# QingzhiWang/LIS-SLAM

Measured on AMD Instinct MI355X. Metric: scan-to-submap registrations/sec (64x1800 pts, 200k submap), higher is better.
Workload: dtype f32; 1 GPU; configs[1]: batch=64 synthetic 64x1800 scans vs one shared 200k-pt submap per GPU, semantic mask off, 10 fixed GN iterations, target index build inside the step; batch_per_gpu=64, submap_points=200000, gn_iters=10, parallelism=independent batches x1 + RCCL all-gather of results

## Files before the change

### include/lisreg.h

```cpp
#ifndef LISREG_H_
#define LISREG_H_

#include <stdint.h>

#ifdef __cplusplus
extern "C" {
#endif

#define LISREG_VERSION 1

#define LISREG_OK                        0
#define LISREG_NOT_ENOUGH_FEATURES       1
#define LISREG_TOO_FEW_CORRESPONDENCES   2
#define LISREG_LEAF_TOO_SMALL            3
#define LISREG_ERR_ARG                  -1
#define LISREG_ERR_HIP                  -2
#define LISREG_ERR_NO_TARGET            -3
#define LISREG_ERR_NOMEM                -4
#define LISREG_ERR_COMM                 -5

#define LISREG_FMT_XYZI    0
#define LISREG_FMT_XYZIL   1
#define LISREG_FMT_DEVICE  2
#define LISREG_FMT_DEVICE_XYZI 4
// ... 88 lines not shown
int  lisreg_batch_prepare(lisreg_ctx* ctx, int n_items, const lisreg_item* items,
                          const lisreg_params* params, const float* T_init);
int  lisreg_batch_run(lisreg_ctx* ctx);
int  lisreg_batch_fetch(lisreg_ctx* ctx, float* T, lisreg_stats* stats);
int  lisreg_stage_host_items(lisreg_ctx* ctx, int n_items, const lisreg_item* items, lisreg_item* items_out);

void* lisreg_batch_result_device(const lisreg_ctx* ctx);

int  lisreg_set_option(lisreg_ctx* ctx, const char* name, int value);
int  lisreg_get_option(const lisreg_ctx* ctx, const char* name, int* value);

int  lisreg_get_counters(lisreg_ctx* ctx, unsigned long long* out, int n);

int  lisreg_get_neighbors(lisreg_ctx* ctx, int* out, int n_elems);

int  lisreg_test_fit_models(lisreg_ctx* ctx, int kind, int n, const float* neighbours, const float* queries,
                            const lisreg_params* params, int exact, float* out);

#define LISREG_SOLVE_STATE_STRIDE 56
int  lisreg_test_solve_steps(lisreg_ctx* ctx, int n_items, int n_steps, const int* n_rows, const double* rows,
                             const float* T_init, const int* degenerate_in, const int* n_sc, const int* n_ss,
                             const lisreg_imu* imu, const lisreg_params* params,
                             float* trace_out, float* state_out, float* results_out);

int  lisreg_get_target_index(lisreg_ctx* ctx, int slot, int kind, int* dims, float* geom,
                             float* sorted_out, int sorted_capacity, int* cell_start_out, int cell_capacity);

int  lisreg_get_target_graph(lisreg_ctx* ctx, int slot, int kind, int* k, float* rows_out, float* meta_out, int capacity_points);

int  lisreg_get_target_cell_rows(lisreg_ctx* ctx, int slot, int kind, int* n_rows, int* k, int* table_out, int capacity_cells,
                                 float* rows_out, float* meta_out, int capacity_rows);

int  lisreg_get_trace(lisreg_ctx* ctx, float* buf, int max_iters);

int  lisreg_set_profiling(lisreg_ctx* ctx, int enable);
int  lisreg_get_timing(lisreg_ctx* ctx, double out[5]);

int  lisreg_voxel_downsample(lisreg_ctx* ctx, const void* in, int n, int stride_bytes, int fmt, float leaf,
                             void* out, int out_capacity, int* n_out);
int  lisreg_voxel_downsample_multi(lisreg_ctx* ctx, int k, const void* const* in, const int* n, const float* leaf, int fmt,
                                   void* const* out, const int* out_capacity, int* n_out);
int  lisreg_transform_cloud(lisreg_ctx* ctx, const void* in, int n, int stride_bytes, int fmt, const float T[6], void* out);

#define LISREG_FMT_XYZIRT  3
typedef struct lisreg_feature_params {
    int   n_scan;
// ... 325 lines not shown
```

### lis-slam_amd/csrc/lisreg_api.hip

```cpp
#include "lisreg_ctx.hpp"

#include <dlfcn.h>

#include <algorithm>
#include <chrono>
#include <cmath>
#include <cstdio>
#include <cstdlib>
#include <cstring>
#include <string>
#include <vector>

using namespace lisreg;

namespace lisreg {
thread_local std::string g_static_err;
int ctx_fail(lisreg_ctx* c, int code, const std::string& msg)
{
    if (c) c->err = msg; else g_static_err = msg;
    return code;
}

bool ensure_side_stream(lisreg_ctx* c)
{
// ... 1349 lines not shown
    return LISREG_OK;
}

int lisreg_test_fit_models(lisreg_ctx* c, int kind, int n, const float* neighbours, const float* queries, const lisreg_params* params,
                           int exact, float* out)
{
    if (!c) return LISREG_ERR_ARG;
    if ((kind != 0 && kind != 1) || n < 0 || !params || (n > 0 && (!neighbours || !queries || !out)))
        return fail(c, LISREG_ERR_ARG, "test_fit_models: bad arguments");
    if (n == 0) return LISREG_OK;
    HIPCHK(c, hipSetDevice(c->device));
    DevBuf nb, q, o;
    HIPCHK(c, nb.ensure(sizeof(float) * 15 * (size_t)n));
    HIPCHK(c, q.ensure(sizeof(float) * 3 * (size_t)n));
    HIPCHK(c, o.ensure(sizeof(float) * 10 * (size_t)n));
    HIPCHK(c, hipMemcpyAsync(nb.p, neighbours, sizeof(float) * 15 * (size_t)n, hipMemcpyHostToDevice, c->stream));
    HIPCHK(c, hipMemcpyAsync(q.p, queries, sizeof(float) * 3 * (size_t)n, hipMemcpyHostToDevice, c->stream));
    DevParams prm = make_dev_params(*params);
    prm.exact = exact ? 1 : 0;
    if (exact) launch_test_fit_exact(kind, n, nb.as<float>(), q.as<float>(), prm, o.as<float>(), c->stream);
    else launch_test_fit(kind, n, nb.as<float>(), q.as<float>(), prm, o.as<float>(), c->stream);
    HIPCHK(c, hipGetLastError());
    HIPCHK(c, hipMemcpyAsync(out, o.p, sizeof(float) * 10 * (size_t)n, hipMemcpyDeviceToHost, c->stream));
    HIPCHK(c, hipStreamSynchronize(c->stream));
    return LISREG_OK;
}

int lisreg_test_solve_steps(lisreg_ctx* c, int n_items, int n_steps, const int* n_rows, const double* rows, const float* T_init,
                            const int* degenerate_in, const int* n_sc, const int* n_ss, const lisreg_imu* imu,
                            const lisreg_params* params, float* trace_out, float* state_out, float* results_out)
{
    if (!c) return LISREG_ERR_ARG;
    if (n_items < 0 || n_steps < 1 || n_steps > 64 || !params || (n_items > 0 && (!n_rows || !T_init)))
        return fail(c, LISREG_ERR_ARG, "test_solve_steps: bad arguments");
    if (n_items == 0) return LISREG_OK;
    size_t total_rows = 0;
    for (int i = 0; i < n_items; ++i) {
        if (n_rows[i] < 0) return fail(c, LISREG_ERR_ARG, "test_solve_steps: negative row count");
        total_rows += (size_t)n_rows[i];
    }
    if (total_rows > 0x7fffffffu || (total_rows > 0 && !rows)) return fail(c, LISREG_ERR_ARG, "test_solve_steps: bad rows");
    HIPCHK(c, hipSetDevice(c->device));
    const size_t n = (size_t)n_items;
    DevParams prm = make_dev_params(*params);
    std::vector<ItemState> h_items(n);
    memset(h_items.data(), 0, sizeof(ItemState) * n);
// ... 694 lines not shown
```

### lis-slam_amd/csrc/lisreg_index.hip

```cpp
#include "lisreg_internal.hpp"

namespace lisreg {

namespace {

constexpr int kScanBlock = 256;
constexpr int kScanItems = 8;
constexpr int kScanTile  = kScanBlock * kScanItems;

__device__ __forceinline__ int wave_incl_scan(int v, int lane)
{
#pragma unroll
    for (int d = 1; d < 64; d <<= 1) {
        int t = __shfl_up(v, d);
        if (lane >= d) v += t;
    }
    return v;
}

__device__ __forceinline__ int block_excl_scan(int v, int* total, int* s_wave )
{
    const int lane = threadIdx.x & 63, wave = threadIdx.x >> 6;
    int inc = wave_incl_scan(v, lane);
    if (lane == 63) s_wave[wave] = inc;
// ... 561 lines not shown
    if (!kLarge || n_s <= cap) {
        SlotsLds sl;
        sl.idx = (uint32_t*)(s_dyn + ucap + 1);
        sl.pos = (uint16_t*)(sl.idx + cap);
        strip_build_body<NT>(t, y0, cell0, ucells, s0, n_s, s_dyn, sl, tmp_pts, s_wave);
    } else {
        SlotsGlobal sl;
        sl.idx = g_slot_idx + s0; sl.pos = g_slot_pos + s0;
        strip_build_body<NT>(t, y0, cell0, ucells, s0, n_s, s_dyn, sl, tmp_pts, s_wave);
    }
}

constexpr int kGraphWPB = 1;
constexpr int kGraphPPW = 8;

template <int M> __device__ __forceinline__ int lane_xor(int v)
{
    if constexpr (M == 1)       return __builtin_amdgcn_mov_dpp(v, 0xB1, 0xF, 0xF, true);
    else if constexpr (M == 2)  return __builtin_amdgcn_mov_dpp(v, 0x4E, 0xF, 0xF, true);
    else if constexpr (M == 3)  return __builtin_amdgcn_mov_dpp(v, 0x1B, 0xF, 0xF, true);
    else if constexpr (M == 7)  return __builtin_amdgcn_mov_dpp(v, 0x141, 0xF, 0xF, true);
    else if constexpr (M == 15) return __builtin_amdgcn_mov_dpp(v, 0x140, 0xF, 0xF, true);
    else if constexpr (M == 8)  return __builtin_amdgcn_mov_dpp(v, 0x128, 0xF, 0xF, true);
    else return __shfl_xor(v, M);
}

__device__ __forceinline__ void graph_row_q32(const GridIndex& g, const float4 q, int hx, int hy, int hz, int s,
                                              float4* __restrict__ row_out, float2* __restrict__ meta_out, int (*s_off)[64], int (*s_js)[64]);

__device__ __forceinline__ void graph_build_wave(const GridIndex& g, int s, int (*s_off)[64], int (*s_js)[64])
{
    const float4 q = g.pts[s];
    const int hx = cell_coord(q.x, g.ox, g.inv_cell, g.nx), hy = cell_coord(q.y, g.oy, g.inv_cell, g.ny), hz = cell_coord(q.z, g.oz, g.inv_cell, g.nz);
    graph_row_q32(g, q, hx, hy, hz, s, const_cast<float4*>(g.nbr) + (size_t)s * kGraphK, const_cast<float2*>(g.nbr_meta) + s, s_off, s_js);
}

__global__ __launch_bounds__(64 * kGraphWPB) void k_graph_build_one(GridIndex g)
{
    __shared__ int s_off[kGraphWPB][64], s_js[kGraphWPB][64];
    const int first = (blockIdx.x * kGraphWPB + (threadIdx.x >> 6)) * kGraphPPW;
#pragma unroll 1
    for (int i = 0; i < kGraphPPW; ++i) {
        const int s = first + i;
        if (s >= g.n) break;
        graph_build_wave(g, s, s_off, s_js);
    }
}
// ... 139 lines not shown
    for (int dx = -2; dx <= 2; ++dx) {
        const int x = ix + dx;
        if (x < 0 || x >= g.nx) continue;
#pragma unroll
        for (int dy = -2; dy <= 2; ++dy) {
            const int y = iy + dy;
            if (y < 0 || y >= g.ny) continue;
            const int base = (x * g.ny + y) * g.nz;
            cnt5 += g.cell_start[base + z1 + 1] - g.cell_start[base + z0];
        }
    }
    const int m = omask[cid] & 255;
    const bool r = cnt5 != 0 && crow_reached(g, reach, ix, iy, iz);
    need[cid] = r ? 1 + __popc(m) : 0;
    omask[cid] = cnt5 ? (r ? (m | (min(cnt5, 0xffff) << 8)) : kCrowUnreached) : 0;
}

__global__ __launch_bounds__(256) void k_crow_classify_plain(GridIndex g, int n_cells, int* __restrict__ need, int* __restrict__ omask,
                                                             const unsigned* __restrict__ reach)
{
    crow_classify_plain_body(g, n_cells, need, omask, reach, blockIdx.x);
}

template <int M, int LowBit> __device__ __forceinline__ unsigned cmpx32(unsigned k, int lane)
{
    const unsigned pk = (unsigned)lane_xor<M>((int)k);
    const unsigned lo = min(k, pk), hi = max(k, pk);
    return (lane & LowBit) == 0 ? lo : hi;
}
template <int H> __device__ __forceinline__ unsigned half_cleaners32(unsigned k, int lane)
{
    if constexpr (H > 0) { k = cmpx32<H, H>(k, lane); return half_cleaners32<(H >> 1)>(k, lane); }
    else return k;
}
template <int H> __device__ __forceinline__ unsigned merge_blocks32(unsigned k, int lane)
{
    k = cmpx32<2 * H - 1, H>(k, lane);
    return half_cleaners32<(H >> 1)>(k, lane);
}
__device__ __forceinline__ unsigned sort64x32(unsigned k, int lane)
{
    k = merge_blocks32<1>(k, lane); k = merge_blocks32<2>(k, lane); k = merge_blocks32<4>(k, lane);
    k = merge_blocks32<8>(k, lane); k = merge_blocks32<16>(k, lane); k = merge_blocks32<32>(k, lane);
    return k;
}

template <int R>
struct CrowBlock { int x0, x1, y0, y1, z0, z1, total; };

template <int R>
__device__ __forceinline__ CrowBlock<R> crow_runs(const GridIndex& g, int hx, int hy, int hz, int (*s_off)[64], int (*s_js)[64])
{
    constexpr int W = 2 * R + 1, NR = W * W;
    static_assert(NR <= 64, "one lane per z-run");
    const int lane = threadIdx.x & 63, wave = threadIdx.x >> 6;
    CrowBlock<R> b;
    b.x0 = max(hx - R, 0); b.x1 = min(hx + R, g.nx - 1); b.y0 = max(hy - R, 0); b.y1 = min(hy + R, g.ny - 1);
    b.z0 = max(hz - R, 0); b.z1 = min(hz + R, g.nz - 1);
    int js = 0, len = 0;
    if (lane < NR) {
        const int ix = hx + lane / W - R, iy = hy + lane % W - R;
        if (ix >= b.x0 && ix <= b.x1 && iy >= b.y0 && iy <= b.y1) {
            const int base = (ix * g.ny + iy) * g.nz;
            js = g.cell_start[base + b.z0];
            len = g.cell_start[base + b.z1 + 1] - js;
        }
    }
    int inc = len;
#pragma unroll
    for (int d = 1; d < 64; d <<= 1) { const int t = __shfl_up(inc, d); if (lane >= d) inc += t; }
    b.total = __shfl(inc, 63);
    __builtin_amdgcn_wave_barrier();
    s_off[wave][lane] = inc - len; s_js[wave][lane] = js;
    __builtin_amdgcn_wave_barrier();
    return b;
}

template <int R>
__device__ __forceinline__ float crow_inscribed(const GridIndex& g, const CrowBlock<R>& b, float qx, float qy, float qz)
{
    float rc = 3.0e18f;
    if (b.x0 > 0)        rc = fminf(rc, qx - (g.ox + (float)b.x0 * g.cell));
    if (b.x1 < g.nx - 1) rc = fminf(rc, (g.ox + (float)(b.x1 + 1) * g.cell) - qx);
    if (b.y0 > 0)        rc = fminf(rc, qy - (g.oy + (float)b.y0 * g.cell));
    if (b.y1 < g.ny - 1) rc = fminf(rc, (g.oy + (float)(b.y1 + 1) * g.cell) - qy);
    if (b.z0 > 0)        rc = fminf(rc, qz - (g.oz + (float)b.z0 * g.cell));
    if (b.z1 < g.nz - 1) rc = fminf(rc, (g.oz + (float)(b.z1 + 1) * g.cell) - qz);
    return fmaxf(rc - 1e-3f, 0.f);
}

constexpr unsigned kInfQ = 0x7f800000u;

constexpr int kListQueueWaves = 4;
template <int R, bool kFilter = false>
__device__ __forceinline__ void crow_list(const GridIndex& g, const CrowBlock<R>& b, float qx, float qy, float qz,
                                          int (*s_off)[64], int (*s_js)[64], unsigned& topk, int& topi, float4& topc, bool& have_c,
                                          int exclude = -1 ,
                                          float rc2 = 3.0e38f )
{
    constexpr int W = 2 * R + 1, NR = W * W;
    const int lane = threadIdx.x & 63, wave = threadIdx.x >> 6;
    __shared__ unsigned s_qk[kListQueueWaves][128];
    __shared__ int s_qj[kListQueueWaves][128];
    topk = kInfQ; topi = -1;
    topc = make_float4(0.f, 0.f, 0.f, 0.f);
    have_c = b.total <= 64;
    auto candidate = [&](int t, int& cj, float4& cc) -> unsigned {
        unsigned ck = kInfQ;
        cj = -1; cc = make_float4(0.f, 0.f, 0.f, 0.f);
        if (t < b.total) {
            int lo = 0, hi = NR - 1;
#pragma unroll
            for (int it = 0; it < (NR > 32 ? 6 : 5); ++it) { const int mid = (lo + hi + 1) >> 1; if (s_off[wave][mid] <= t) lo = mid; else hi = mid - 1; }
            const int j = s_js[wave][lo] + (t - s_off[wave][lo]);
            const float4 c = g.pts[j];
            cc = c;
            const float ex = qx - c.x, ey = qy - c.y, ez = qz - c.z;
            const float d2 = ex * ex + ey * ey + ez * ez;
            if (j != exclude && d2 < 3.0e38f) { ck = __float_as_uint(d2) & ~0x7Fu; cj = j; }
        }
        return ck;
    };
    bool first = true;
    auto take = [&](unsigned ck_in, int cj, const float4 cc) {
        unsigned k = ck_in | (unsigned)lane;
        k = sort64x32(k, lane);
        const int cs = __shfl(cj, (int)(k & 63u));
        const unsigned ck = k & ~0x7Fu;
        if (have_c) { const int sl = (int)(k & 63u); topc = make_float4(__shfl(cc.x, sl), __shfl(cc.y, sl), __shfl(cc.z, sl), 0.f); }
        if (first) { topk = ck; topi = cs; first = false; }
        else {
            const unsigned kt = topk | 64u | (unsigned)lane;
            const unsigned kcr = (unsigned)__shfl((int)(ck | (unsigned)lane), 63 - lane);
            const unsigned m = half_cleaners32<32>(min(kt, kcr), lane);
            const int pos = (int)(m & 63u);
            const int from_top = __shfl(topi, pos), from_chunk = __shfl(cs, pos);
            topi = (m & 64u) ? from_top : from_chunk;
            topk = m & ~0x7Fu;
        }
    };
    if (!kFilter || b.total <= 64) {
#pragma unroll 1
        for (int c0 = 0; c0 < b.total; c0 += 64) {
            int cj; float4 cc;
            const unsigned ck = candidate(c0 + lane, cj, cc);
            take(ck, cj, cc);
        }
        return;
    }
    int pend = 0;
#pragma unroll 1
    for (int c0 = 0; c0 < b.total; c0 += 64) {
        int cj; float4 cc;
        const unsigned ck = candidate(c0 + lane, cj, cc);
        const bool in = cj >= 0 && __uint_as_float(ck) <= rc2;
        const unsigned long long m = __ballot(in);
        if (in) {
            const int slot = pend + (int)__builtin_amdgcn_mbcnt_hi((unsigned)(m >> 32), __builtin_amdgcn_mbcnt_lo((unsigned)m, 0u));
            s_qk[wave][slot] = ck; s_qj[wave][slot] = cj;
        }
        pend += __popcll(m);
        __builtin_amdgcn_wave_barrier();
        if (pend >= 64) {
            const unsigned qk = s_qk[wave][lane]; const int qj = s_qj[wave][lane];
            const int rest = pend - 64;
            unsigned rk = 0u; int rj = 0;
            if (lane < rest) { rk = s_qk[wave][64 + lane]; rj = s_qj[wave][64 + lane]; }
            __builtin_amdgcn_wave_barrier();
            if (lane < rest) { s_qk[wave][lane] = rk; s_qj[wave][lane] = rj; }
            pend = rest;
            __builtin_amdgcn_wave_barrier();
            take(qk, qj, make_float4(0.f, 0.f, 0.f, 0.f));
        }
    }
    if (pend > 0 || first) {
        unsigned qk = kInfQ; int qj = -1;
        if (lane < pend) { qk = s_qk[wave][lane]; qj = s_qj[wave][lane]; }
// ... 67 lines not shown
                const int oi = __shfl(keep ? topi : -1, sl);
                const float ox = __shfl(e.x, sl), oy = __shfl(e.y, sl), oz = __shfl(e.z, sl);
                const bool okeep = oi >= 0 && __uint_as_float(k & ~0x7Fu) <= rho_o2;
                const int ocnt = __popcll(__ballot(okeep));
                float4 oe = make_float4(mx, my, mz, __int_as_float(-1));
                if (okeep) oe = make_float4(ox, oy, oz, __int_as_float(oi));
                orow[lane] = oe;
                if (lane == 0) meta_out[slot] = make_float2(rho_o2, __int_as_float(ocnt));
            } else {
                unsigned ok; int oi; bool okeep; float4 oe, oc; bool ohave;
                const float orc = crow_inscribed<R>(g, b, mx, my, mz);
                crow_list<R>(g, b, mx, my, mz, s_off, s_js, ok, oi, oc, ohave, -1, orc * orc);
                (void)crow_emit(g, mx, my, mz, orc, ok, oi, orow, meta_out + slot, okeep, oe, oc, ohave);
            }
            ++slot;
        }
    }
}

constexpr int kCrowWPB = 1;
constexpr int kCrowCPW = 8;
constexpr int kCrowWaves = 6;
static_assert(kGraphWPB <= kListQueueWaves && kCrowWPB <= kListQueueWaves, "crow_list's LDS queue has one region per wavefront of a workgroup");
__device__ __forceinline__ void crow_build_body(const GridIndex& g, int n_cells, const int* __restrict__ need, int* __restrict__ omask,
                                                const int* __restrict__ scan, int cap,
                                                int blk_, int (*s_off)[64], int (*s_js)[64])
{
    const int lane = threadIdx.x & 63;
    const int first = __builtin_amdgcn_readfirstlane((blk_ * kCrowWPB + (int)(threadIdx.x >> 6)) * kCrowCPW);
    int* tab = const_cast<int*>(g.crow_tab);
    int n_l = 0, b_l = 0, om_l = 0;
    if (lane < kCrowCPW && first + lane < n_cells) {
        n_l = need[first + lane];
        om_l = omask[first + lane];
        omask[first + lane] = 0;
        if (n_l) b_l = scan[first + lane];
        const bool fits = n_l != 0 && !(b_l + n_l > cap || b_l >= (1 << 23));
        tab[first + lane] = n_l == 0 ? ((om_l & kCrowUnreached) ? -1 : -2) : (fits ? (b_l << 8) | (om_l & 255) : -1);
        if (!fits) n_l = 0;
    }
    unsigned long long live = __ballot(n_l != 0);
#pragma unroll 1
    while (live) {
        const int i = __ffsll((long long)live) - 1;
        live &= live - 1;
        const int cid = first + i;
// ... 20 lines not shown
__global__ __launch_bounds__(256) void k_crow_mark_pair(CrowJobs J, float margin_cells)
{
    const int k = (int)blockIdx.x < J.j[0].nb ? 0 : 1;
    const CrowJob& j = J.j[k];
    crow_mark_body(j.g, margin_cells * j.g.cell, j.omask, (int)blockIdx.x - (k ? J.j[0].nb : 0));
}
__global__ __launch_bounds__(256) void k_crow_classify_pair(CrowJobs J, float margin_cells)
{
    extern __shared__ int s_cs[];
    const int k = (int)blockIdx.x < J.j[0].nb ? 0 : 1;
    const CrowJob& j = J.j[k];
    const int blk = (int)blockIdx.x - (k ? J.j[0].nb : 0);
    if (j.plain) crow_classify_plain_body(j.g, j.n_cells, j.need, j.omask, j.reach, blk);
    else crow_classify_body(j.g, j.tiles_y, j.need, j.omask, j.reach, blk, s_cs, margin_cells * j.g.cell);
}
__global__ __launch_bounds__(64 * kCrowWPB) __attribute__((amdgpu_waves_per_eu(kCrowWaves, kCrowWaves))) void k_crow_build_pair(CrowJobs J)
{
    __shared__ int s_off[kCrowWPB][64], s_js[kCrowWPB][64];
    const int k = (int)blockIdx.x < J.j[0].nb ? 0 : 1;
    const CrowJob& j = J.j[k];
    crow_build_body(j.g, j.n_cells, j.need, j.omask, j.scan, j.cap, (int)blockIdx.x - (k ? J.j[0].nb : 0), s_off, s_js);
}

__global__ __launch_bounds__(kBlockQ) void k_count_jumps(const BlockDesc* __restrict__ blocks, const Segment* __restrict__ segs,
                                                         float thr2, int* __restrict__ jumps)
{
    const BlockDesc bd = blocks[blockIdx.x];
    const Segment sg = segs[bd.seg];
    const int e = bd.start + threadIdx.x;
    bool jump = false;
    if ((int)threadIdx.x < bd.count && e + 1 < sg.n) {
        const float4 a = sg.src[e], b = sg.src[e + 1];
        const float dx = a.x - b.x, dy = a.y - b.y, dz = a.z - b.z;
        jump = dx * dx + dy * dy + dz * dz > thr2;
    }
    const unsigned long long m = __ballot(jump);
    if ((threadIdx.x & 63) == 0 && m) atomicAdd(jumps, __popcll(m));
}

__global__ __launch_bounds__(256) void k_voxel_keys(const float4* __restrict__ pts, int n, VoxelDesc d,
                                                    uint32_t* __restrict__ elem_bucket, uint32_t* __restrict__ elem_sub,
                                                    int* __restrict__ hist)
{
    const int i = blockIdx.x * 256 + threadIdx.x;
    if (i >= n) return;
    const float4 p = pts[i];
// ... 569 lines not shown
    if (m.off[m.k] > 0) k_concat_jobs<<<(m.off[m.k] + 255) / 256, 256, 0, st>>>(j, m, cat);
}

__global__ void k_multi_bounds(const int* __restrict__ slot, VoxelMulti m, int* __restrict__ out)
{
    if ((int)threadIdx.x <= m.k) out[threadIdx.x] = slot[m.off[threadIdx.x]];
}
void launch_multi_bounds(const int* slot, const VoxelMulti& m, int* out, hipStream_t st) { k_multi_bounds<<<1, 64, 0, st>>>(slot, m, out); }

__global__ __launch_bounds__(256) void k_hand_out(const float4* __restrict__ src, VoxelHandOut h)
{
    const int v = blockIdx.x * 256 + threadIdx.x;
    if (v >= h.vo[h.k]) return;
    int s = 0;
#pragma unroll
    for (int j = 1; j < kVoxelMultiMax; ++j) if (j < h.k && v >= h.vo[j]) s = j;
    h.out[s][v - h.vo[s]] = src[v];
}
void launch_hand_out(const float4* src, const VoxelHandOut& h, hipStream_t st)
{
    if (h.vo[h.k] > 0) k_hand_out<<<(h.vo[h.k] + 255) / 256, 256, 0, st>>>(src, h);
}

void launch_count_jumps(const BlockDesc* blocks, int n_blocks, const Segment* segs, float thr, int* jumps, hipStream_t st)
{
    (void)hipMemsetAsync(jumps, 0, sizeof(int), st);
    if (n_blocks > 0) k_count_jumps<<<n_blocks, kBlockQ, 0, st>>>(blocks, segs, thr * thr, jumps);
}

void launch_exclusive_scan(const int* in, int* out, int* tmp, int n, hipStream_t st) { exclusive_scan(in, out, tmp, n, st); }

void launch_pack_cloud(const void* raw_dev, size_t n, int stride, int has_label, float4* out, hipStream_t st)
{
    if (n > 0) k_pack_cloud<<<(unsigned)((n + 255) / 256), 256, 0, st>>>(static_cast<const unsigned char*>(raw_dev), n, stride, has_label, out);
}

void launch_transform_cloud(const float4* in, int n, const float* M12_dev, float4* out, hipStream_t st)
{
    if (n > 0) k_transform_cloud<<<(n + 255) / 256, 256, 0, st>>>(in, n, M12_dev, out);
}
void launch_transform_cloud_m(const float4* in, int n, const float M12_host[12], float4* out, hipStream_t st)
{
    Mat12 M;
    for (int i = 0; i < 12; ++i) M.m[i] = M12_host[i];
    if (n > 0) k_transform_cloud_m<<<(n + 255) / 256, 256, 0, st>>>(in, n, M, out);
}
// ... 3 lines not shown
```

### lis-slam_amd/csrc/lisreg_internal.hpp

```cpp
#pragma once
#include <hip/hip_runtime.h>
#include <stdint.h>
#include "../../include/lisreg.h"

namespace lisreg {

constexpr int kBlockQ     = 256;
constexpr int kNumAcc     = 28;
constexpr int kResultSize = 12;
constexpr int kTraceStride = LISREG_TRACE_STRIDE;
constexpr int kGraphK     = 64;

struct GridIndex {
    const float4* pts;
    const int*    cell_start;
    int   n;
    float ox, oy, oz;
    float cell, inv_cell;
    int   nx, ny, nz;
    const float4* nbr;
    const float2* nbr_meta;
    const float4* crow;
    const float2* crow_meta;
    const int*    crow_tab;
// ... 132 lines not shown
void launch_sort_sources(const BlockDesc* blocks, int n_blocks, const Segment* segs, int n_segs,
                         const ItemState* items, int n_elems, int n_buckets, SortBuffers sb, float4* sorted_all, int* order_all,
                         hipStream_t st);
void launch_reset_items(ItemState* items, int n_items, DevParams prm, int* done_counter, hipStream_t st, int* zero_too = nullptr);
void launch_assoc(const BlockDesc* blocks, int n_blocks, const Segment* segs, const GridIndex* grids,
                  const ItemState* items, DevParams prm, const float4* sorted_all, double* partials,
                  int mode ,
                  int* nn, int n_elems, float first_pass_r2,
                  bool wide ,
                  int graph_hops ,
                  unsigned long long* counters ,
                  int* dbg_nn ,
                  int lanes_q ,
                  const BlockDesc* blocks_q, int n_blocks_q ,
                  float4* coef, int* coef_ok ,
                  const int* xcd_order , hipStream_t st);
void launch_assoc_exact(const BlockDesc* blocks, int n_blocks, const Segment* segs, const GridIndex* grids,
                        const ItemState* items, DevParams prm, const float4* sorted_all, double* partials,
                        int mode, int* nn, int n_elems, float first_pass_r2, bool wide, int graph_hops,
                        unsigned long long* counters, int* dbg_nn, int lanes_q, const BlockDesc* blocks_q, int n_blocks_q,
                        float4* coef, int* coef_ok, const int* xcd_order, hipStream_t st);
void launch_test_fit(int kind, int n, const float* nb15, const float* q3, DevParams prm, float* out, hipStream_t st);
void launch_test_fit_exact(int kind, int n, const float* nb15, const float* q3, DevParams prm, float* out, hipStream_t st);
void launch_xcd_order(const BlockDesc* blocks, int n_blocks, const Segment* segs, const GridIndex* grids, const ItemState* items,
                      const float4* sorted_all, bool by_target, int* keys, int* order, hipStream_t st);
void launch_pose_gather(const ItemState* items, int n_items, float* T_out, hipStream_t st);
void launch_pose_cache_from_trig(ItemState* items, int n_items, const float* trig, hipStream_t st);
void launch_solve(ItemState* items, int n_items, DevParams prm, const double* partials, float* trace,
                  int trace_cap, int* done_counter, hipStream_t st);
void launch_finalize(ItemState* items, int n_items, DevParams prm, float* results, hipStream_t st, int* reset_done_counter = nullptr);

void launch_voxel_sort(const float4* pts, int n, VoxelDesc d, int n_buckets, SortBuffers sb, int* order, uint32_t* sidx,
                       int* head, int* slot , hipStream_t st);
struct VoxelHandOut { int k; int vo[kVoxelMultiMax + 1]; float4* out[kVoxelMultiMax]; };
void launch_bbox_multi(const float4* cat, const VoxelMulti& m, float* bbox_out , float* scratch , hipStream_t st);
struct BboxJobs { int k; int n[kVoxelMultiMax]; const float4* pts[kVoxelMultiMax]; };
void launch_bbox_jobs(const BboxJobs& j, float* bbox_out , float* scratch , hipStream_t st);
struct CloudRef { const float4* pts; int n; int pad_; };
void launch_bbox_refs(const CloudRef* refs_dev, int k, float* bbox_out , float* scratch , hipStream_t st);
void launch_concat_jobs(const BboxJobs& j, const VoxelMulti& m, float4* cat, hipStream_t st);
void launch_multi_bounds(const int* slot, const VoxelMulti& m, int* out , hipStream_t st);
void launch_hand_out(const float4* src, const VoxelHandOut& h, hipStream_t st);
void launch_voxel_sort_multi(const float4* pts, int n, const VoxelMulti& m, int n_buckets, SortBuffers sb, int* order, uint32_t* sidx,
                             int* head, int* slot, hipStream_t st);
void launch_voxel_centroids(int n, int n_vox, const float4* pts, const uint32_t* labels, int w_mode, const int* order,
                            const int* head, const int* slot, int* vstart , float4* out_pts,
// ... 90 lines not shown
```

### lis-slam_amd/lisreg/__init__.py

```python
from __future__ import annotations

import ctypes as C
import os
import subprocess

import numpy as np

_PKG = os.path.dirname(os.path.dirname(os.path.abspath(__file__)))
LIB_PATH = os.path.join(_PKG, "lib", "liblisreg.so")
CSRC = os.path.join(_PKG, "csrc")

OK, NOT_ENOUGH_FEATURES, TOO_FEW_CORRESPONDENCES, LEAF_TOO_SMALL = 0, 1, 2, 3
ERR_ARG, ERR_HIP, ERR_NO_TARGET, ERR_NOMEM, ERR_COMM = -1, -2, -3, -4, -5
FMT_XYZI, FMT_XYZIL, FMT_DEVICE, FMT_XYZIRT, FMT_DEVICE_XYZI, FMT_XYZI_PACKED = 0, 1, 2, 3, 4, 5
VARIANT_ODOM, VARIANT_KEYFRAME, VARIANT_SUBMAP = 1, 2, 3
TRACE_STRIDE = 56
RESULT_SIZE = 12
SOLVE_STATE_STRIDE = 56

ABI_SYMBOLS = [
    "lisreg_device_count", "lisreg_create", "lisreg_destroy", "lisreg_last_error", "lisreg_set_stream",
    "lisreg_get_stream", "lisreg_default_params", "lisreg_set_target", "lisreg_set_target_slot",
    "lisreg_target_from_classes", "lisreg_align", "lisreg_align_batch", "lisreg_batch_prepare", "lisreg_batch_run",
    "lisreg_batch_fetch", "lisreg_stage_host_items", "lisreg_upload_cloud", "lisreg_concat_device", "lisreg_batch_result_device", "lisreg_set_option", "lisreg_get_option", "lisreg_get_counters", "lisreg_get_neighbors", "lisreg_test_fit_models", "lisreg_test_solve_steps", "lisreg_get_target_index", "lisreg_get_target_graph", "lisreg_get_target_cell_rows", "lisreg_keyframes_reset", "lisreg_keyframes_push", "lisreg_keyframes_target", "lisreg_get_trace",
    "lisreg_set_profiling", "lisreg_get_timing", "lisreg_pose_to_matrix", "lisreg_transform_update",
    "lisreg_comm_unique_id", "lisreg_comm_init", "lisreg_gather_results", "lisreg_comm_destroy",
    "lisreg_voxel_downsample", "lisreg_voxel_downsample_multi", "lisreg_transform_cloud",
    "lisreg_extract_features", "lisreg_extract_features_deskew", "lisreg_extract_features_batch", "lisreg_default_feature_params", "lisreg_semantic_split",
    "lisreg_map_index_set", "lisreg_map_index_set_batch", "lisreg_nearest", "lisreg_dynamic_filter", "lisreg_bbx_filter", "lisreg_cloud_bounds",
    "lisreg_localmap_default_params", "lisreg_localmap_reset", "lisreg_localmap_insert", "lisreg_localmap_extract",
    "lisreg_localmap_get", "lisreg_predict_pose", "lisreg_guess_state_init", "lisreg_update_initial_guess", "lisreg_submap_insert", "lisreg_submap_extract", "lisreg_submap_crop_boxes",
    "lisreg_default_gather_params", "lisreg_submap_gather_count", "lisreg_submap_gather",
    "lisreg_icp_default_params", "lisreg_icp_align", "lisreg_icp_align_batch", "lisreg_icp_gn_match",
    "lisreg_loopdet_default_params", "lisreg_loopdet_reset", "lisreg_loopdet_detect", "lisreg_loopdet_candidates",
    "lisreg_loopdet_get", "lisreg_loop_descriptor",
    "lisreg_loopdet_configure", "lisreg_loopdet_matches", "lisreg_loopdet_candidate_scores", "lisreg_loopdet_get_descriptor",
    "lisreg_loop_descriptor_kind",
    "lisreg_default_pretreat_params", "lisreg_pretreat", "lisreg_pretreat_batch",
    "lisreg_default_rangenet_params", "lisreg_rangenet_project", "lisreg_rangenet_project_batch", "lisreg_rangenet_label",
    "lisreg_rangenet_label_batch",
]


ICP_NOT_CONVERGED, ICP_ITERATIONS, ICP_TRANSFORM, ICP_ABS_MSE, ICP_REL_MSE, ICP_NO_CORRESPONDENCES = range(6)


class IcpParams(C.Structure):
# ... 239 lines not shown
        L.lisreg_get_stream.argtypes = [vp]
        L.lisreg_get_stream.restype = vp
        L.lisreg_default_params.argtypes = [C.c_int, C.POINTER(Params)]
        L.lisreg_set_target.argtypes = [vp, vp, C.c_int, vp, C.c_int, C.c_int, C.c_int]
        L.lisreg_set_target_slot.argtypes = [vp, C.c_int, vp, C.c_int, vp, C.c_int, C.c_int, C.c_int]
        L.lisreg_target_from_classes.argtypes = [vp, C.c_int, vp, C.c_int, vp, C.c_int, vp, C.c_int, vp, C.c_int,
                                                 C.c_int, C.c_int]
        L.lisreg_align.argtypes = [vp, vp, C.c_int, vp, C.c_int, C.c_int, C.c_int, C.POINTER(Params),
                                   C.POINTER(Imu), fp, C.POINTER(Stats)]
        L.lisreg_align_batch.argtypes = [vp, C.c_int, C.POINTER(Item), C.POINTER(Params), fp, C.POINTER(Stats)]
        L.lisreg_batch_prepare.argtypes = [vp, C.c_int, C.POINTER(Item), C.POINTER(Params), fp]
        L.lisreg_stage_host_items.argtypes = [vp, C.c_int, C.POINTER(Item), C.POINTER(Item)]
        L.lisreg_batch_run.argtypes = [vp]
        L.lisreg_batch_fetch.argtypes = [vp, fp, C.POINTER(Stats)]
        L.lisreg_batch_result_device.argtypes = [vp]
        L.lisreg_batch_result_device.restype = vp
        L.lisreg_set_option.argtypes = [vp, C.c_char_p, C.c_int]
        L.lisreg_upload_cloud.argtypes = [vp, vp, C.c_int, C.c_int, C.c_int, vp]
        L.lisreg_concat_device.argtypes = [vp, C.c_int, C.POINTER(C.c_void_p), C.POINTER(C.c_int), vp, C.POINTER(C.c_int)]
        L.lisreg_get_option.argtypes = [vp, C.c_char_p, C.POINTER(C.c_int)]
        L.lisreg_get_neighbors.argtypes = [vp, C.POINTER(C.c_int), C.c_int]
        if hasattr(L, "lisreg_test_fit_models"): L.lisreg_test_fit_models.argtypes = [vp, C.c_int, C.c_int, C.POINTER(C.c_float), C.POINTER(C.c_float), C.POINTER(Params), C.c_int, C.POINTER(C.c_float)]
        if hasattr(L, "lisreg_test_solve_steps"): L.lisreg_test_solve_steps.argtypes = [vp, C.c_int, C.c_int, ip, C.POINTER(C.c_double), fp, ip, ip, ip, C.POINTER(Imu), C.POINTER(Params), fp, fp, fp]
        L.lisreg_get_target_index.argtypes = [vp, C.c_int, C.c_int, C.POINTER(C.c_int), C.POINTER(C.c_float), C.c_void_p, C.c_int, C.c_void_p, C.c_int]
        L.lisreg_get_target_graph.argtypes = [vp, C.c_int, C.c_int, C.POINTER(C.c_int), C.POINTER(C.c_float), C.POINTER(C.c_float), C.c_int]
        L.lisreg_get_target_cell_rows.argtypes = [vp, C.c_int, C.c_int, C.POINTER(C.c_int), C.POINTER(C.c_int), C.POINTER(C.c_int), C.c_int,
                                                  C.POINTER(C.c_float), C.POINTER(C.c_float), C.c_int]
        L.lisreg_get_counters.argtypes = [vp, C.POINTER(C.c_ulonglong), C.c_int]
        L.lisreg_get_trace.argtypes = [vp, fp, C.c_int]
        L.lisreg_set_profiling.argtypes = [vp, C.c_int]
        L.lisreg_get_timing.argtypes = [vp, C.POINTER(C.c_double)]
        L.lisreg_pose_to_matrix.argtypes = [fp, fp]
        L.lisreg_pose_to_matrix.restype = None
        L.lisreg_transform_update.argtypes = [C.POINTER(Params), C.POINTER(Imu), fp]
        L.lisreg_transform_update.restype = None
        L.lisreg_comm_unique_id.argtypes = [C.POINTER(C.c_ubyte)]
        L.lisreg_comm_init.argtypes = [vp, C.c_int, C.c_int, C.POINTER(C.c_ubyte)]
        L.lisreg_gather_results.argtypes = [vp, vp, C.c_int, vp]
        L.lisreg_comm_destroy.argtypes = [vp]
        L.lisreg_comm_destroy.restype = None
        L.lisreg_voxel_downsample_multi.argtypes = [vp, C.c_int, C.POINTER(C.c_void_p), C.POINTER(C.c_int), C.POINTER(C.c_float), C.c_int,
                                                    C.POINTER(C.c_void_p), C.POINTER(C.c_int), C.POINTER(C.c_int)]
        L.lisreg_voxel_downsample.argtypes = [vp, vp, C.c_int, C.c_int, C.c_int, C.c_float, vp, C.c_int, ip]
        L.lisreg_transform_cloud.argtypes = [vp, vp, C.c_int, C.c_int, C.c_int, fp, vp]
        L.lisreg_extract_features.argtypes = [vp, vp, C.c_int, C.c_int, C.c_int, C.POINTER(FeatureParams), C.POINTER(FeatureOut)]
        L.lisreg_default_feature_params.argtypes = [C.POINTER(FeatureParams)]
# ... 208 lines not shown
        n = len(n_rows); total = int(n_rows.sum())
        rows = np.ascontiguousarray(rows, np.float64)
        assert rows.ndim == 3 and rows.shape[1:] == (total, 28), rows.shape
        n_steps = rows.shape[0]
        T0 = np.ascontiguousarray(T_init, np.float32).reshape(n, 6)
        ip, fp = C.POINTER(C.c_int), C.POINTER(C.c_float)
        opt = lambda a: None if a is None else np.ascontiguousarray(a, np.int32).reshape(n)
        deg, sc, ss = opt(degenerate_in), opt(n_sc), opt(n_ss)
        iptr = lambda a: None if a is None else a.ctypes.data_as(ip)
        imu_arr = None
        if imu is not None:
            imu_arr = (Imu * max(n, 1))()
            for i, m in enumerate(imu):
                if m is not None:
                    imu_arr[i] = m
        trace = np.zeros((n, n_steps, TRACE_STRIDE), np.float32)
        state = np.zeros((n, n_steps, SOLVE_STATE_STRIDE), np.float32)
        results = np.zeros((n, RESULT_SIZE), np.float32)
        self._chk(self._L.lisreg_test_solve_steps(self._h, n, n_steps, n_rows.ctypes.data_as(ip), rows.ctypes.data_as(C.POINTER(C.c_double)),
                                                  T0.ctypes.data_as(fp), iptr(deg), iptr(sc), iptr(ss), imu_arr, C.byref(params),
                                                  trace.ctypes.data_as(fp), state.ctypes.data_as(fp), results.ctypes.data_as(fp)))
        return dict(trace=trace, state=state, results=results)

    def front_end(self) -> int:
        return self.get_option("front_end")

    def set_profiling_paused(self, paused: bool):
        self._chk(self._L.lisreg_set_profiling(self._h, 0 if paused else 1))

    def set_target(self, corner: np.ndarray, surf: np.ndarray, slot: int = 0):
        corner = np.ascontiguousarray(corner); surf = np.ascontiguousarray(surf)
        self._chk(self._L.lisreg_set_target_slot(self._h, slot, _vp(corner), len(corner), _vp(surf), len(surf),
                                                 corner.dtype.itemsize, _fmt_of(corner)))

    def set_target_device(self, corner_ptr: int, n_corner: int, surf_ptr: int, n_surf: int, slot: int = 0):
        self._chk(self._L.lisreg_set_target_slot(self._h, slot, C.c_void_p(corner_ptr), n_corner,
                                                 C.c_void_p(surf_ptr), n_surf, 16, FMT_DEVICE))

    def target_from_classes(self, pole, ground, building, dynamic, slot: int = 0):
        arrs = [np.ascontiguousarray(a) for a in (pole, ground, building, dynamic)]
        self._chk(self._L.lisreg_target_from_classes(self._h, slot, _vp(arrs[0]), len(arrs[0]), _vp(arrs[1]),
                                                     len(arrs[1]), _vp(arrs[2]), len(arrs[2]), _vp(arrs[3]),
                                                     len(arrs[3]), arrs[0].dtype.itemsize, _fmt_of(arrs[0])))

    def align(self, src_corner: np.ndarray, src_surf: np.ndarray, T_init, params: Params, imu: Imu | None = None):
        sc = np.ascontiguousarray(src_corner); ss = np.ascontiguousarray(src_surf)
# ... 852 lines not shown
```

Measured before the change: 30230 registrations/s.

## Use DPP and permlane swaps for wave scans, sorts and run lookup

Replaces the shfl_up-based wave prefix sum with a DPP row-shift/broadcast scan. The bitonic sort's 16- and 32-lane stages now use permlane16/32 swaps with XOR flipping, and the top-k merge is factored into list_take, which sorts descending for later chunks so the cross-lane reversal shuffle is gone. The per-lane binary search over cell offsets in crow_list becomes a ballot plus LDS scatter and DPP max-scan. This cuts LDS traffic and cross-lane latency in neighbour-list construction, at the cost of relying on gfx950-specific permlane builtins; a test entry point for these lane ops is also added.

Result: no change. 30460 registrations/s, median of 6 (+0.7%).

```diff
diff --git a/include/lisreg.h b/include/lisreg.h
--- a/include/lisreg.h
+++ b/include/lisreg.h
@@ -134,6 +134,10 @@
                              const float* T_init, const int* degenerate_in, const int* n_sc, const int* n_ss,
                              const lisreg_imu* imu, const lisreg_params* params,
                              float* trace_out, float* state_out, float* results_out);
+
+#define LISREG_LANE_OPS_MERGE_IN (8 + 4 * 128)
+#define LISREG_LANE_OPS_RUN_IN (8 + 128)
+int  lisreg_test_lane_ops(lisreg_ctx* ctx, int kind, int n_waves, const int* in, int* out);
 
 int  lisreg_get_target_index(lisreg_ctx* ctx, int slot, int kind, int* dims, float* geom,
                              float* sorted_out, int sorted_capacity, int* cell_start_out, int cell_capacity);
diff --git a/lis-slam_amd/csrc/lisreg_api.hip b/lis-slam_amd/csrc/lisreg_api.hip
--- a/lis-slam_amd/csrc/lisreg_api.hip
+++ b/lis-slam_amd/csrc/lisreg_api.hip
@@ -1395,6 +1395,34 @@
     else launch_test_fit(kind, n, nb.as<float>(), q.as<float>(), prm, o.as<float>(), c->stream);
     HIPCHK(c, hipGetLastError());
     HIPCHK(c, hipMemcpyAsync(out, o.p, sizeof(float) * 10 * (size_t)n, hipMemcpyDeviceToHost, c->stream));
+    HIPCHK(c, hipStreamSynchronize(c->stream));
+    return LISREG_OK;
+}
+
+int lisreg_test_lane_ops(lisreg_ctx* c, int kind, int n_waves, const int* in, int* out)
+{
+    if (!c) return LISREG_ERR_ARG;
+    if (kind < 0 || kind > 3 || n_waves < 0 || n_waves > (1 << 20) || (n_waves > 0 && (!in || !out)))
+        return fail(c, LISREG_ERR_ARG, "test_lane_ops: bad arguments");
+    if (n_waves == 0) return LISREG_OK;
+    const size_t n_in = (size_t)n_waves * (kind == 1 ? kLaneOpsMergeIn : kind == 3 ? kLaneOpsRunIn : 64);
+    const size_t n_out = (size_t)n_waves * (kind == 0 ? 64 : 128);
+    if (kind == 1 || kind == 3)
+        for (int w = 0; w < n_waves; ++w) {
+            const int h = in[(size_t)w * (kind == 1 ? kLaneOpsMergeIn : kLaneOpsRunIn)];
+            const int* hd = in + (size_t)w * kLaneOpsRunIn;
+            if (kind == 1 ? (h < 1 || h > 4) : ((h != 25 && h != 49) || hd[1] < 0 || hd[8] != 0))
+                return fail(c, LISREG_ERR_ARG, "test_lane_ops: bad case header");
+        }
+    HIPCHK(c, hipSetDevice(c->device));
+    DevBuf i, o;
+    HIPCHK(c, i.ensure(sizeof(int) * n_in));
+    HIPCHK(c, o.ensure(sizeof(int) * n_out));
+    HIPCHK(c, hipMemcpyAsync(i.p, in, sizeof(int) * n_in, hipMemcpyHostToDevice, c->stream));
+    HIPCHK(c, hipMemsetAsync(o.p, 0, sizeof(int) * n_out, c->stream));
+    launch_test_lane_ops(kind, n_waves, i.as<int>(), o.as<int>(), c->stream);
+    HIPCHK(c, hipGetLastError());
+    HIPCHK(c, hipMemcpyAsync(out, o.p, sizeof(int) * n_out, hipMemcpyDeviceToHost, c->stream));
     HIPCHK(c, hipStreamSynchronize(c->stream));
     return LISREG_OK;
 }
diff --git a/lis-slam_amd/csrc/lisreg_index.hip b/lis-slam_amd/csrc/lisreg_index.hip
--- a/lis-slam_amd/csrc/lisreg_index.hip
+++ b/lis-slam_amd/csrc/lisreg_index.hip
@@ -607,7 +607,27 @@
     else if constexpr (M == 7)  return __builtin_amdgcn_mov_dpp(v, 0x141, 0xF, 0xF, true);
     else if constexpr (M == 15) return __builtin_amdgcn_mov_dpp(v, 0x140, 0xF, 0xF, true);
     else if constexpr (M == 8)  return __builtin_amdgcn_mov_dpp(v, 0x128, 0xF, 0xF, true);
+    else if constexpr (M == 4)  return __builtin_amdgcn_mov_dpp(__builtin_amdgcn_mov_dpp(v, 0x141, 0xF, 0xF, true), 0x1B, 0xF, 0xF, true);
     else return __shfl_xor(v, M);
+}
+
+template <bool kMax> __device__ __forceinline__ int wave_scan_dpp(int v)
+{
+    constexpr int id = kMax ? (int)0x80000000 : 0;
+    auto op = [](int a, int b) { return kMax ? max(a, b) : a + b; };
+    v = op(v, __builtin_amdgcn_update_dpp(id, v, 0x111, 0xF, 0xF, false));
+    v = op(v, __builtin_amdgcn_update_dpp(id, v, 0x112, 0xF, 0xF, false));
+    v = op(v, __builtin_amdgcn_update_dpp(id, v, 0x114, 0xF, 0xF, false));
+    v = op(v, __builtin_amdgcn_update_dpp(id, v, 0x118, 0xF, 0xF, false));
+    v = op(v, __builtin_amdgcn_update_dpp(id, v, 0x142, 0xA, 0xF, false));
+    v = op(v, __builtin_amdgcn_update_dpp(id, v, 0x143, 0xC, 0xF, false));
+    return v;
+}
+__device__ __forceinline__ int wave_incl_sum(int v, int& total)
+{
+    v = wave_scan_dpp<false>(v);
+    total = __builtin_amdgcn_readlane(v, 63);
+    return v;
 }
 
 __device__ __forceinline__ void graph_row_q32(const GridIndex& g, const float4 q, int hx, int hy, int hz, int s,
@@ -793,8 +813,16 @@
     crow_classify_plain_body(g, n_cells, need, omask, reach, blockIdx.x);
 }
 
+typedef unsigned int v2u_lane __attribute__((ext_vector_type(2)));
 template <int M, int LowBit> __device__ __forceinline__ unsigned cmpx32(unsigned k, int lane)
 {
+    if constexpr (M == 16 || M == 32) {
+        static_assert(LowBit == M, "a half cleaner's step");
+        v2u_lane r;
+        if constexpr (M == 16) r = __builtin_amdgcn_permlane16_swap(k, k, false, false);
+        else r = __builtin_amdgcn_permlane32_swap(k, k, false, false);
+        return (lane & LowBit) == 0 ? min(r.x, r.y) : max(r.x, r.y);
+    }
     const unsigned pk = (unsigned)lane_xor<M>((int)k);
     const unsigned lo = min(k, pk), hi = max(k, pk);
     return (lane & LowBit) == 0 ? lo : hi;
@@ -811,9 +839,49 @@
 }
 __device__ __forceinline__ unsigned sort64x32(unsigned k, int lane)
 {
+    const unsigned f16 = (unsigned)((int)((unsigned)lane << 26) >> 31);
+    const unsigned f8 = (unsigned)((int)(((unsigned)lane ^ ((unsigned)lane << 1)) << 26) >> 31);
+    k ^= f8;
     k = merge_blocks32<1>(k, lane); k = merge_blocks32<2>(k, lane); k = merge_blocks32<4>(k, lane);
-    k = merge_blocks32<8>(k, lane); k = merge_blocks32<16>(k, lane); k = merge_blocks32<32>(k, lane);
+    k = merge_blocks32<8>(k, lane);
+    k ^= f8 ^ f16;
+    k = half_cleaners32<16>(k, lane);
+    k ^= f16;
+    k = half_cleaners32<32>(k, lane);
     return k;
+}
+
+__device__ __forceinline__ int list_take(unsigned& topk, int& topi, bool first, unsigned ck_in, int cj, int lane)
+{
+    unsigned k = ck_in | (unsigned)lane;
+    const unsigned flip = first ? 0u : ~0u;
+    k = sort64x32(k ^ flip, lane) ^ flip;
+    const int sl = (int)(k & 63u);
+    if (first) { topk = k & ~0x7Fu; topi = __shfl(cj, sl); return sl; }
+    const unsigned kt = topk | 64u | (unsigned)lane;
+    const unsigned m = half_cleaners32<32>(min(kt, k), lane);
+    const int pos = (int)(m & 63u);
+    const int from_top = __shfl(topi, pos), from_chunk = __shfl(cj, pos);
+    topi = (m & 64u) ? from_top : from_chunk;
+    topk = m & ~0x7Fu;
+    return sl;
+}
+
+template <int NR>
+__device__ __forceinline__ int crow_run_of(const int* s_off_w, int* s_run_w, int c0, int lane)
+{
+    static_assert(NR < 64, "s_off[NR] is read");
+    int o0 = 0x7fffffff, o1 = 0x7fffffff;
+    if (lane < NR) { o0 = s_off_w[lane]; o1 = s_off_w[lane + 1]; }
+    const int r0 = __popcll(__ballot(o0 <= c0)) - 1;
+    __builtin_amdgcn_wave_barrier();
+    s_run_w[lane] = -1;
+    __builtin_amdgcn_wave_barrier();
+    if (o1 > o0 && (unsigned)(o0 - c0) < 64u) s_run_w[o0 - c0] = lane;
+    __builtin_amdgcn_wave_barrier();
+    const int v = wave_scan_dpp<true>(s_run_w[lane]);
+    __builtin_amdgcn_wave_barrier();
+    return max(v, r0);
 }
 
 template <int R>
@@ -837,10 +905,7 @@
             len = g.cell_start[base + b.z1 + 1] - js;
         }
     }
-    int inc = len;
-#pragma unroll
-    for (int d = 1; d < 64; d <<= 1) { const int t = __shfl_up(inc, d); if (lane >= d) inc += t; }
-    b.total = __shfl(inc, 63);
+    const int inc = wave_incl_sum(len, b.total);
     __builtin_amdgcn_wave_barrier();
     s_off[wave][lane] = inc - len; s_js[wave][lane] = js;
     __builtin_amdgcn_wave_barrier();
@@ -862,6 +927,7 @@
 
 constexpr unsigned kInfQ = 0x7f800000u;
 
+constexpr int kRunWaves = 1;
 constexpr int kListQueueWaves = 4;
 template <int R, bool kFilter = false>
 __device__ __forceinline__ void crow_list(const GridIndex& g, const CrowBlock<R>& b, float qx, float qy, float qz,
@@ -873,17 +939,17 @@
     const int lane = threadIdx.x & 63, wave = threadIdx.x >> 6;
     __shared__ unsigned s_qk[kListQueueWaves][128];
     __shared__ int s_qj[kListQueueWaves][128];
+    __shared__ int s_run[kRunWaves][64];
     topk = kInfQ; topi = -1;
     topc = make_float4(0.f, 0.f, 0.f, 0.f);
     have_c = b.total <= 64;
-    auto candidate = [&](int t, int& cj, float4& cc) -> unsigned {
+    auto candidate = [&](int c0, int& cj, float4& cc) -> unsigned {
         unsigned ck = kInfQ;
         cj = -1; cc = make_float4(0.f, 0.f, 0.f, 0.f);
+        const int t = c0 + lane;
+        const int run = crow_run_of<NR>(s_off[wave], s_run[wave], c0, lane);
         if (t < b.total) {
-            int lo = 0, hi = NR - 1;
-#pragma unroll
-            for (int it = 0; it < (NR > 32 ? 6 : 5); ++it) { const int mid = (lo + hi + 1) >> 1; if (s_off[wave][mid] <= t) lo = mid; else hi = mid - 1; }
-            const int j = s_js[wave][lo] + (t - s_off[wave][lo]);
+            const int j = s_js[wave][run] + (t - s_off[wave][run]);
             const float4 c = g.pts[j];
             cc = c;
             const float ex = qx - c.x, ey = qy - c.y, ez = qz - c.z;
@@ -894,27 +960,15 @@
     };
     bool first = true;
     auto take = [&](unsigned ck_in, int cj, const float4 cc) {
-        unsigned k = ck_in | (unsigned)lane;
-        k = sort64x32(k, lane);
-        const int cs = __shfl(cj, (int)(k & 63u));
-        const unsigned ck = k & ~0x7Fu;
-        if (have_c) { const int sl = (int)(k & 63u); topc = make_float4(__shfl(cc.x, sl), __shfl(cc.y, sl), __shfl(cc.z, sl), 0.f); }
-        if (first) { topk = ck; topi = cs; first = false; }
-        else {
-            const unsigned kt = topk | 64u | (unsigned)lane;
-            const unsigned kcr = (unsigned)__shfl((int)(ck | (unsigned)lane), 63 - lane);
-            const unsigned m = half_cleaners32<32>(min(kt, kcr), lane);
-            const int pos = (int)(m & 63u);
-            const int from_top = __shfl(topi, pos), from_chunk = __shfl(cs, pos);
-            topi = (m & 64u) ? from_top : from_chunk;
-            topk = m & ~0x7Fu;
-        }
+        const int sl = list_take(topk, topi, first, ck_in, cj, lane);
+        if (have_c) topc = make_float4(__shfl(cc.x, sl), __shfl(cc.y, sl), __shfl(cc.z, sl), 0.f);
+        first = false;
     };
     if (!kFilter || b.total <= 64) {
 #pragma unroll 1
         for (int c0 = 0; c0 < b.total; c0 += 64) {
             int cj; float4 cc;
-            const unsigned ck = candidate(c0 + lane, cj, cc);
+            const unsigned ck = candidate(c0, cj, cc);
             take(ck, cj, cc);
         }
         return;
@@ -923,7 +977,7 @@
 #pragma unroll 1
     for (int c0 = 0; c0 < b.total; c0 += 64) {
         int cj; float4 cc;
-        const unsigned ck = candidate(c0 + lane, cj, cc);
+        const unsigned ck = candidate(c0, cj, cc);
         const bool in = cj >= 0 && __uint_as_float(ck) <= rc2;
         const unsigned long long m = __ballot(in);
         if (in) {
@@ -1037,6 +1091,7 @@
 constexpr int kCrowCPW = 8;
 constexpr int kCrowWaves = 6;
 static_assert(kGraphWPB <= kListQueueWaves && kCrowWPB <= kListQueueWaves, "crow_list's LDS queue has one region per wavefront of a workgroup");
+static_assert(kGraphWPB <= kRunWaves && kCrowWPB <= kRunWaves, "crow_run_of's LDS region: one per wavefront of a workgroup");
 __device__ __forceinline__ void crow_build_body(const GridIndex& g, int n_cells, const int* __restrict__ need, int* __restrict__ omask,
                                                 const int* __restrict__ scan, int cap,
                                                 int blk_, int (*s_off)[64], int (*s_js)[64])
@@ -1103,6 +1158,37 @@
     crow_build_body(j.g, j.n_cells, j.need, j.omask, j.scan, j.cap, (int)blockIdx.x - (k ? J.j[0].nb : 0), s_off, s_js);
 }
 
+__global__ __launch_bounds__(64) void k_test_lane_ops(int kind, const int* __restrict__ in, int* __restrict__ out)
+{
+    __shared__ int s_off[1][64], s_js[1][64], s_run[1][64];
+    const int lane = threadIdx.x & 63, w = blockIdx.x;
+    if (kind == 0) {
+        out[w * 64 + lane] = (int)sort64x32((unsigned)in[w * 64 + lane], lane);
+    } else if (kind == 1) {
+        const int* cin = in + (size_t)w * kLaneOpsMergeIn;
+        const int n_chunks = cin[0];
+        unsigned topk = kInfQ; int topi = -1;
+        for (int c = 0; c < n_chunks; ++c)
+            (void)list_take(topk, topi, c == 0, (unsigned)cin[8 + c * 128 + lane], cin[8 + c * 128 + 64 + lane], lane);
+        out[w * 128 + lane] = (int)topk; out[w * 128 + 64 + lane] = topi;
+    } else if (kind == 2) {
+        const int len = in[w * 64 + lane];
+        int total;
+        const int inc = wave_incl_sum(len, total);
+        out[w * 128 + lane] = inc - len;
+        if (lane == 0) out[w * 128 + 64] = total;
+    } else {
+        const int* cin = in + (size_t)w * kLaneOpsRunIn;
+        const int nr = cin[0], c0 = cin[1], total = cin[2];
+        s_off[0][lane] = cin[8 + lane]; s_js[0][lane] = cin[8 + 64 + lane];
+        __builtin_amdgcn_wave_barrier();
+        const int run = nr == 25 ? crow_run_of<25>(s_off[0], s_run[0], c0, lane) : crow_run_of<49>(s_off[0], s_run[0], c0, lane);
+        const int t = c0 + lane;
+        const bool has = t < total;
+        out[w * 128 + lane] = has ? run : -1;
+        out[w * 128 + 64 + lane] = has ? s_js[0][run] + (t - s_off[0][run]) : -1;
+    }
+}
 __global__ __launch_bounds__(kBlockQ) void k_count_jumps(const BlockDesc* __restrict__ blocks, const Segment* __restrict__ segs,
                                                          float thr2, int* __restrict__ jumps)
 {
@@ -1718,6 +1804,11 @@
     if (h.vo[h.k] > 0) k_hand_out<<<(h.vo[h.k] + 255) / 256, 256, 0, st>>>(src, h);
 }
 
+void launch_test_lane_ops(int kind, int n_waves, const int* in, int* out, hipStream_t st)
+{
+    if (n_waves > 0) k_test_lane_ops<<<n_waves, 64, 0, st>>>(kind, in, out);
+}
+
 void launch_count_jumps(const BlockDesc* blocks, int n_blocks, const Segment* segs, float thr, int* jumps, hipStream_t st)
 {
     (void)hipMemsetAsync(jumps, 0, sizeof(int), st);
diff --git a/lis-slam_amd/csrc/lisreg_internal.hpp b/lis-slam_amd/csrc/lisreg_internal.hpp
--- a/lis-slam_amd/csrc/lisreg_internal.hpp
+++ b/lis-slam_amd/csrc/lisreg_internal.hpp
@@ -178,6 +178,8 @@
                         float4* coef, int* coef_ok, const int* xcd_order, hipStream_t st);
 void launch_test_fit(int kind, int n, const float* nb15, const float* q3, DevParams prm, float* out, hipStream_t st);
 void launch_test_fit_exact(int kind, int n, const float* nb15, const float* q3, DevParams prm, float* out, hipStream_t st);
+constexpr int kLaneOpsMergeIn = 8 + 4 * 128, kLaneOpsRunIn = 8 + 128;
+void launch_test_lane_ops(int kind, int n_waves, const int* in, int* out, hipStream_t st);
 void launch_xcd_order(const BlockDesc* blocks, int n_blocks, const Segment* segs, const GridIndex* grids, const ItemState* items,
                       const float4* sorted_all, bool by_target, int* keys, int* order, hipStream_t st);
 void launch_pose_gather(const ItemState* items, int n_items, float* T_out, hipStream_t st);
diff --git a/lis-slam_amd/lisreg/__init__.py b/lis-slam_amd/lisreg/__init__.py
--- a/lis-slam_amd/lisreg/__init__.py
+++ b/lis-slam_amd/lisreg/__init__.py
@@ -17,12 +17,14 @@
 TRACE_STRIDE = 56
 RESULT_SIZE = 12
 SOLVE_STATE_STRIDE = 56
+LANE_OPS_MERGE_IN = 8 + 4 * 128
+LANE_OPS_RUN_IN = 8 + 128
 
 ABI_SYMBOLS = [
     "lisreg_device_count", "lisreg_create", "lisreg_destroy", "lisreg_last_error", "lisreg_set_stream",
     "lisreg_get_stream", "lisreg_default_params", "lisreg_set_target", "lisreg_set_target_slot",
     "lisreg_target_from_classes", "lisreg_align", "lisreg_align_batch", "lisreg_batch_prepare", "lisreg_batch_run",
-    "lisreg_batch_fetch", "lisreg_stage_host_items", "lisreg_upload_cloud", "lisreg_concat_device", "lisreg_batch_result_device", "lisreg_set_option", "lisreg_get_option", "lisreg_get_counters", "lisreg_get_neighbors", "lisreg_test_fit_models", "lisreg_test_solve_steps", "lisreg_get_target_index", "lisreg_get_target_graph", "lisreg_get_target_cell_rows", "lisreg_keyframes_reset", "lisreg_keyframes_push", "lisreg_keyframes_target", "lisreg_get_trace",
+    "lisreg_batch_fetch", "lisreg_stage_host_items", "lisreg_upload_cloud", "lisreg_concat_device", "lisreg_batch_result_device", "lisreg_set_option", "lisreg_get_option", "lisreg_get_counters", "lisreg_get_neighbors", "lisreg_test_fit_models", "lisreg_test_solve_steps", "lisreg_test_lane_ops", "lisreg_get_target_index", "lisreg_get_target_graph", "lisreg_get_target_cell_rows", "lisreg_keyframes_reset", "lisreg_keyframes_push", "lisreg_keyframes_target", "lisreg_get_trace",
     "lisreg_set_profiling", "lisreg_get_timing", "lisreg_pose_to_matrix", "lisreg_transform_update",
     "lisreg_comm_unique_id", "lisreg_comm_init", "lisreg_gather_results", "lisreg_comm_destroy",
     "lisreg_voxel_downsample", "lisreg_voxel_downsample_multi", "lisreg_transform_cloud",
@@ -308,6 +310,7 @@
         L.lisreg_get_neighbors.argtypes = [vp, C.POINTER(C.c_int), C.c_int]
         if hasattr(L, "lisreg_test_fit_models"): L.lisreg_test_fit_models.argtypes = [vp, C.c_int, C.c_int, C.POINTER(C.c_float), C.POINTER(C.c_float), C.POINTER(Params), C.c_int, C.POINTER(C.c_float)]
         if hasattr(L, "lisreg_test_solve_steps"): L.lisreg_test_solve_steps.argtypes = [vp, C.c_int, C.c_int, ip, C.POINTER(C.c_double), fp, ip, ip, ip, C.POINTER(Imu), C.POINTER(Params), fp, fp, fp]
+        if hasattr(L, "lisreg_test_lane_ops"): L.lisreg_test_lane_ops.argtypes = [vp, C.c_int, C.c_int, ip, ip]
         L.lisreg_get_target_index.argtypes = [vp, C.c_int, C.c_int, C.POINTER(C.c_int), C.POINTER(C.c_float), C.c_void_p, C.c_int, C.c_void_p, C.c_int]
         L.lisreg_get_target_graph.argtypes = [vp, C.c_int, C.c_int, C.POINTER(C.c_int), C.POINTER(C.c_float), C.POINTER(C.c_float), C.c_int]
         L.lisreg_get_target_cell_rows.argtypes = [vp, C.c_int, C.c_int, C.POINTER(C.c_int), C.POINTER(C.c_int), C.POINTER(C.c_int), C.c_int,
@@ -562,6 +565,15 @@
                                                   trace.ctypes.data_as(fp), state.ctypes.data_as(fp), results.ctypes.data_as(fp)))
         return dict(trace=trace, state=state, results=results)
 
+    def test_lane_ops(self, kind: int, cases: np.ndarray) -> np.ndarray:
+        a = np.ascontiguousarray(cases).view(np.int32)
+        width = {0: 64, 1: LANE_OPS_MERGE_IN, 2: 64, 3: LANE_OPS_RUN_IN}[int(kind)]
+        assert a.ndim == 2 and a.shape[1] == width, a.shape
+        out = np.zeros((a.shape[0], 64 if kind == 0 else 128), np.int32)
+        ip = C.POINTER(C.c_int)
+        self._chk(self._L.lisreg_test_lane_ops(self._h, int(kind), a.shape[0], a.ctypes.data_as(ip), out.ctypes.data_as(ip)))
+        return out
+
     def front_end(self) -> int:
         return self.get_option("front_end")
 
```
